# MariusFurter/WeightedSampling.jl

Hardware: NVIDIA B200
Metric: particle_updates_per_sec (higher is better)
Workload: dtype f64

## Files before the change

### weightedsampling.jl_b200/csrc/ws_internal.h

```cpp
#pragma once
#include <cuda_runtime.h>
#include <stdint.h>
#include "ws_vm.cuh"
#include "ws_mailbox.cuh"

#ifndef WS_VM_BLOCK
#define WS_VM_BLOCK 128
#endif
#ifndef WS_VM_P
#define WS_VM_P 3
#endif
#ifndef WS_VM_MINB
#define WS_VM_MINB 5
#endif
#define WS_VM_MAX_IO 24
#define WS_VM_MAX_CKPT 16
#define WS_VM_MAX_OPS 96
#define WS_VM_MAX_REGS ((192 * 1024) / (WS_VM_BLOCK * WS_VM_P * 8))
#define WS_SCAN_BLOCK 256
#define WS_SCAN_ITEMS 8
#define WS_SCAN_TILE (32 * WS_SCAN_ITEMS)
#define WS_CDF_TILE (WS_SCAN_BLOCK * WS_SCAN_ITEMS)
#define WS_GATHER_MAX_PLANES 32
#define WS_HEAVY_TILE_SLOTS 32768
// ... 75 lines not shown

struct WsGatherParams {
    int64_t n;
    const int32_t* ancestors;
    int32_t n_planes;
    int32_t pad;
    const double* src[WS_GATHER_MAX_PLANES];
    double* dst[WS_GATHER_MAX_PLANES];
};

#define WS_COMPOSE_MAX_CHAIN 24
struct WsComposeParams {
    int64_t n;
    int64_t n_rows;
    int32_t n_chain;
    int32_t pad;
    const int32_t* chain[WS_COMPOSE_MAX_CHAIN];
};

cudaError_t ws_launch_vm(const WsVmProgram& P, int grid, cudaStream_t s);
cudaError_t ws_launch_reduce_logw(const double* logw, int64_t n, WsLse* partials, int grid, cudaStream_t s);
cudaError_t ws_launch_finalize(const WsLse* partials, int n_partials, int k, int64_t n_global, double ess_perc_min,
                               WsReduceOut* out, unsigned long long* ties, cudaStream_t s);
#define WS_SMALL_N 4096
cudaError_t ws_launch_resample_small(const WsScanParams& P, const WsLse* partials, int n_partials, double ess_perc_min, WsReduceOut* out,
                                     unsigned long long* ties, int do_finalize, cudaStream_t s);
void ws_scan_set_scale(WsScanParams& P);
size_t ws_scan_words(int64_t n);
cudaError_t ws_launch_scan_search(const WsScanParams& P, int grid, cudaStream_t s);
cudaError_t ws_launch_spacings(const WsScanParams& P, cudaStream_t s);
cudaError_t ws_launch_cdf(const WsScanParams& P, cudaStream_t s);
cudaError_t ws_launch_bounds(const WsScanParams& P, cudaStream_t s);
cudaError_t ws_launch_search(const WsScanParams& P, cudaStream_t s);
cudaError_t ws_launch_finalize_global(const double* all_msq, int n_ranks, int64_t n_global, double ess_perc_min,
                                      WsReduceOut* out, cudaStream_t s, unsigned long long* ties = nullptr);
cudaError_t ws_launch_finalize_mbox(const WsLse* partials, int n_partials, int64_t n_global, double ess_perc_min, WsReduceOut* out,
                                    double* all_msq, unsigned long long* ties, const WsMailbox& M, cudaStream_t s);
cudaError_t ws_launch_cdf_tiles(const WsScanParams& P, cudaStream_t s);
cudaError_t ws_launch_offsets_bounds_mbox(const WsScanParams& P, const WsMailbox& M, unsigned long long* all_tot, const unsigned long long* xmine,
                                          int xw, unsigned long long* xall, cudaStream_t s);
cudaError_t ws_launch_barrier_mbox(const WsMailbox& M, cudaStream_t s);
cudaError_t ws_launch_gather(const WsGatherParams& P, int grid, cudaStream_t s);
cudaError_t ws_launch_fill(double* dst, double v, int64_t n, int grid, cudaStream_t s);
cudaError_t ws_launch_exp_norm(const double* logw, const WsReduceOut* red, double* w, int64_t n, int grid,
                               cudaStream_t s);
cudaError_t ws_launch_sumsq(const double* w, int64_t n, double* partials, int grid, cudaStream_t s);
cudaError_t ws_launch_local_ancestors(int32_t* anc, int64_t n, const int32_t* anc_self, int64_t self_lo, int64_t self_hi,
                                      int64_t spare_base, int grid, cudaStream_t s);
cudaError_t ws_launch_patch_ancestors(int32_t* anc, int64_t n, int64_t self_lo, int64_t self_hi, int64_t spare_base, cudaStream_t s);
struct WsTracedPlane {
    const double* src;
    double* dst;
    int64_t level;
};
cudaError_t ws_launch_trace_rows(const int32_t* anc, int64_t m, const int32_t* const* chain, int n_levels, int64_t n_rows, int32_t* rows,
                                 cudaStream_t s);
cudaError_t ws_launch_push_traced(const WsTracedPlane* planes, int n_planes, int64_t m, const int32_t* rows, cudaStream_t s);
cudaError_t ws_launch_gather_rows(const double* src, const int64_t* idx, int64_t n_idx, double* dst, cudaStream_t s);
cudaError_t ws_launch_compose(const WsComposeParams& P, int32_t* out, const int32_t* start, cudaStream_t s);
cudaError_t ws_launch_compose_rows(const WsComposeParams& P, int64_t* out, const int64_t* start, cudaStream_t s);
int ws_vm_sl_grid(const WsVmProgram& P);
int ws_vm_max_grid(int n_regs, int n_loads, int n_ops, int sm_count, int n_ckpt = 0);
int ws_vm_smem_bytes(int n_regs, int n_loads, int n_ops, int n_ckpt = 0);
cudaError_t ws_kernels_init(int device);
```

### weightedsampling.jl_b200/csrc/ws_kernels.cu

```cuda
#include "ws_internal.h"

static int g_sm_count = 148;

__device__ __forceinline__ void lse_push(WsLse& a, double l) {
    if (l == -INFINITY) return;
    if (l > a.m) {
        double sc = ws_exp_nonpos(a.m - l);
        a.S = a.S * sc + 1.0;
        a.Q = a.Q * sc * sc + 1.0;
        a.m = l;
    } else {
        double e = ws_exp_nonpos(l - a.m);
        a.S += e;
        a.Q += e * e;
    }
}

template <int K>
__device__ __forceinline__ void lse_push_many(WsLse& a, const double (&l)[K], const bool (&live)[K]) {
    double mx = -INFINITY;
#pragma unroll
    for (int j = 0; j < K; ++j)
        if (live[j]) mx = fmax(mx, l[j]);
    if (mx > a.m) {
        const double sc = ws_exp_nonpos(a.m - mx);
        a.S *= sc;
        a.Q *= sc * sc;
        a.m = mx;
    }
#pragma unroll
    for (int j = 0; j < K; ++j) {
        if (live[j] && l[j] != -INFINITY) {
            const double e = ws_exp_nonpos(l[j] - a.m);
// ... 294 lines not shown

    if (P.logw_mode != 0 && P.partials != nullptr) {
        WsLse tot = lse_block_reduce<WS_VM_BLOCK>(part, warp_scratch);
        if (threadIdx.x == 0) P.partials[blockIdx.x] = tot;
    }
    for (int c = 0; CKPT && c < P.n_ckpt; ++c) {
        WsLse st;
        st.m = ck[(c * 3 + 0) * WS_VM_BLOCK];
        st.S = ck[(c * 3 + 1) * WS_VM_BLOCK];
        st.Q = ck[(c * 3 + 2) * WS_VM_BLOCK];
        __syncthreads();
        WsLse tot = lse_block_reduce<WS_VM_BLOCK>(st, warp_scratch);
        if (threadIdx.x == 0) P.ckpt_partials[(size_t)c * gridDim.x + blockIdx.x] = tot;
    }
    if (P.n_expect > 0) {
        __shared__ double esc[WS_VM_BLOCK / 32][8];
        const int lane = threadIdx.x & 31, warp = threadIdx.x >> 5;
#pragma unroll
        for (int k = 0; k < 8; ++k) {
            double v = esum[k];
#pragma unroll
            for (int d = 16; d > 0; d >>= 1) v += __shfl_down_sync(0xffffffffu, v, d);
            if (lane == 0) esc[warp][k] = v;
        }
        __syncthreads();
        if (threadIdx.x < 8 && threadIdx.x < P.n_expect) {
            double v = 0.0;
            for (int w = 0; w < WS_VM_BLOCK / 32; ++w) v += esc[w][threadIdx.x];
            P.expect_partials[(size_t)blockIdx.x * P.n_expect + threadIdx.x] = v;
        }
    }
}

#include "ws_vm_sl.cuh"
#ifndef WS_SL_P
#define WS_SL_P 4
#endif
#ifndef WS_SL_MINB
#define WS_SL_MINB 3
#endif
template <class Sig, int PP>
__global__ void __launch_bounds__(WS_VM_BLOCK, WS_SL_MINB) ws_vm_sl_kernel(const __grid_constant__ WsVmProgram P) {
    extern __shared__ __align__(16) double ws_vm_smem[];
    __shared__ WsLse warp_scratch[WS_VM_BLOCK / 32];
    constexpr int RS = PP * WS_VM_BLOCK;
    constexpr int TILE = WS_VM_BLOCK * PP;
    constexpr int NL = Sig::n_loads, NS = Sig::n_stores;
    double* const stage = ws_vm_smem + threadIdx.x;

    WsLse part;
    part.m = -INFINITY;
    part.S = 0.0;
    part.Q = 0.0;
    const int n = (int)P.n;
    const int n_tiles = (n + TILE - 1) / TILE;
    const bool fired = (P.logw_mode != 3) || P.red->do_resample != 0;
    const int lmode = (P.logw_mode == 3) ? (fired ? 2 : 1) : P.logw_mode;
    const double lbase = (P.logw_mode == 3) ? P.red->log_mean_w : P.logw_base;
    const bool any_gather = P.load_gather != 0u && fired;

    auto tile_index = [&](int tile, int j) -> int {
        const int i = tile * TILE + (int)threadIdx.x + j * WS_VM_BLOCK;
        return i < n ? i : n - 1;
    };
    auto issue_stage = [&](int tile, const int (&anc)[PP]) {
#pragma unroll
        for (int k = 0; k < NL; ++k) {
            const bool g = any_gather && ((P.load_gather >> k) & 1u);
            const double* __restrict__ ptr = P.load_ptr[k];
#pragma unroll
            for (int j = 0; j < PP; ++j)
                ws_cp_async8(stage + k * RS + j * WS_VM_BLOCK, ptr + (unsigned)(g ? anc[j] : tile_index(tile, j)));
        }
        ws_cp_async_commit();
    };
// ... 164 lines not shown
        for (int j = 0; j < PP; ++j)
            if (live[j]) lout[(unsigned)first + j * WS_VM_BLOCK] = lw[j];
    }
#pragma unroll
    for (int c = 0; c < NCK; ++c) {
        if (c < reps) {
            __syncthreads();
            WsLse tot = lse_block_reduce<WS_VM_BLOCK>(st[c], warp_scratch);
            if (threadIdx.x == 0) {
                P.ckpt_partials[(size_t)c * gridDim.x + blockIdx.x] = tot;
                if (c == reps - 1 && P.partials != nullptr) P.partials[blockIdx.x] = tot;
            }
        }
    }
}
static bool ws_slck_ok(const WsVmProgram& P) {
    return P.n_ckpt > 0 && P.n_expect == 0 && (P.logw_mode == 1 || P.logw_mode == 2) && ws_sl_matches_repeated<WsSigLinregObs>(P, WS_SLCK_N);
}
static int ws_slck_grid(const WsVmProgram& P) {
    constexpr int TILE = WS_VM_BLOCK * WS_SLCK_P;
    const int64_t tiles = (P.n + TILE - 1) / TILE;
    const int grid = (int)(tiles < (int64_t)g_sm_count * WS_SLCK_MINB ? tiles : (int64_t)g_sm_count * WS_SLCK_MINB);
    return grid < 1 ? 1 : grid;
}

static bool g_vm_interp_only = false;
template <class Sig>
static cudaError_t ws_launch_vm_sl(const WsVmProgram& P, cudaStream_t s) {
    constexpr int TILE = WS_VM_BLOCK * WS_SL_P;
    const int64_t tiles = (P.n + TILE - 1) / TILE;
    int grid = (int)(tiles < (int64_t)g_sm_count * WS_SL_MINB ? tiles : (int64_t)g_sm_count * WS_SL_MINB);
    if (grid < 1) grid = 1;
    const int smem = (Sig::n_loads > 0 ? Sig::n_loads : 1) * TILE * (int)sizeof(double);
    ws_vm_sl_kernel<Sig, WS_SL_P><<<grid, WS_VM_BLOCK, smem, s>>>(P);
    return cudaGetLastError();
}
int ws_vm_sl_grid(const WsVmProgram& P) {
    if (!g_vm_interp_only && P.n_ckpt != 0 && ws_slck_ok(P)) return ws_slck_grid(P);
    if (g_vm_interp_only || P.n_ckpt != 0 || ws_sl_find(P) < 0) return 0;
    constexpr int TILE = WS_VM_BLOCK * WS_SL_P;
    const int64_t tiles = (P.n + TILE - 1) / TILE;
    int grid = (int)(tiles < (int64_t)g_sm_count * WS_SL_MINB ? tiles : (int64_t)g_sm_count * WS_SL_MINB);
    return grid < 1 ? 1 : grid;
}

static bool ws_vm_staged(int n_regs, int n_loads) {
    return n_loads > 0 && (size_t)(n_regs + n_loads) * WS_VM_BLOCK * WS_VM_P * sizeof(double) <= (size_t)200 * 1024;
}
int ws_vm_smem_bytes(int n_regs, int n_loads, int n_ops, int n_ckpt) {
    const int rows = (n_regs < 1 ? 1 : n_regs) + (ws_vm_staged(n_regs < 1 ? 1 : n_regs, n_loads) ? n_loads : 0);
    return rows * WS_VM_BLOCK * WS_VM_P * (int)sizeof(double) + n_ops * (int)sizeof(WsDop) + n_ckpt * 3 * WS_VM_BLOCK * (int)sizeof(double);
}

int ws_vm_max_grid(int n_regs, int n_loads, int n_ops, int sm_count, int n_ckpt) {
    const int smem = ws_vm_smem_bytes(n_regs, n_loads, n_ops, n_ckpt) + 1024;
    int per_sm = (227 * 1024) / smem;
    if (per_sm > WS_VM_MINB) per_sm = WS_VM_MINB;
    if (per_sm < 1) per_sm = 1;
    return per_sm * sm_count;
}

cudaError_t ws_launch_vm(const WsVmProgram& P, int grid, cudaStream_t s) {
    if (!g_vm_interp_only && P.n_ckpt == 0) {
        switch (ws_sl_find(P)) {
#define WS_SL_CASE(idx, Sig) \
    case idx: return ws_launch_vm_sl<Sig>(P, s);
            WS_SL_SIGS(WS_SL_CASE)
#undef WS_SL_CASE
// ... 5 lines not shown
        ws_vm_sl_ckpt_kernel<WsSigLinregObs, WS_SLCK_P, WS_SLCK_N><<<ws_slck_grid(P), WS_VM_BLOCK, smem_ck, s>>>(P);
        return cudaGetLastError();
    }
    const int smem = ws_vm_smem_bytes(P.n_regs, P.n_loads, P.n_ops, P.n_ckpt);
    if (P.n_ckpt > 0) {
        if (ws_vm_staged(P.n_regs, P.n_loads)) ws_vm_kernel<true, true><<<grid, WS_VM_BLOCK, smem, s>>>(P);
        else ws_vm_kernel<false, true><<<grid, WS_VM_BLOCK, smem, s>>>(P);
    } else if (ws_vm_staged(P.n_regs, P.n_loads)) ws_vm_kernel<true><<<grid, WS_VM_BLOCK, smem, s>>>(P);
    else ws_vm_kernel<false><<<grid, WS_VM_BLOCK, smem, s>>>(P);
    return cudaGetLastError();
}

__global__ void __launch_bounds__(256) ws_reduce_logw_kernel(const double* __restrict__ logw, int64_t n,
                                                             WsLse* __restrict__ partials) {
    __shared__ WsLse warp_scratch[8];
    WsLse part;
    part.m = -INFINITY;
    part.S = 0.0;
    part.Q = 0.0;
    const int64_t stride = (int64_t)gridDim.x * 256;
    for (int64_t i = (int64_t)blockIdx.x * 256 + threadIdx.x; i < n; i += stride) lse_push(part, __ldg(logw + i));
    WsLse tot = lse_block_reduce<256>(part, warp_scratch);
    if (threadIdx.x == 0) partials[blockIdx.x] = tot;
}

cudaError_t ws_launch_reduce_logw(const double* logw, int64_t n, WsLse* partials, int grid, cudaStream_t s) {
    ws_reduce_logw_kernel<<<grid, 256, 0, s>>>(logw, n, partials);
    return cudaGetLastError();
}

__global__ void __launch_bounds__(256) ws_finalize_kernel(const WsLse* __restrict__ partials, int n_partials,
                                                          int64_t n_global, double ess_perc_min,
                                                          WsReduceOut* __restrict__ out, unsigned long long* ties) {
    __shared__ WsLse warp_scratch[8];
    const WsLse tot = lse_block_combine<256>(partials + (size_t)blockIdx.x * n_partials, n_partials, warp_scratch);
    if (threadIdx.x == 0) ws_decide(tot, n_global, ess_perc_min, out + blockIdx.x, ties);
}

cudaError_t ws_launch_finalize(const WsLse* partials, int n_partials, int k, int64_t n_global, double ess_perc_min,
                               WsReduceOut* out, unsigned long long* ties, cudaStream_t s) {
    ws_finalize_kernel<<<k, 256, 0, s>>>(partials, n_partials, n_global, ess_perc_min, out, ties);
    return cudaGetLastError();
}

__global__ void ws_finalize_global_kernel(const double* __restrict__ all_msq, int n_ranks, int64_t n_global,
                                          double ess_perc_min, WsReduceOut* __restrict__ out, unsigned long long* ties) {
    if (threadIdx.x != 0 || blockIdx.x != 0) return;
    ws_decide(lse_combine_ranks(all_msq, n_ranks), n_global, ess_perc_min, out, ties);
}

cudaError_t ws_launch_finalize_global(const double* all_msq, int n_ranks, int64_t n_global, double ess_perc_min,
                                      WsReduceOut* out, cudaStream_t s, unsigned long long* ties) {
    ws_finalize_global_kernel<<<1, 32, 0, s>>>(all_msq, n_ranks, n_global, ess_perc_min, out, ties);
    return cudaGetLastError();
}

__global__ void __launch_bounds__(WS_MBOX_THREADS) ws_finalize_mbox_kernel(const WsLse* __restrict__ partials, int n_partials, int64_t n_global,
                                                                           double ess_perc_min, WsReduceOut* __restrict__ out,
                                                                           double* __restrict__ all_msq, unsigned long long* ties,
                                                                           const __grid_constant__ WsMailbox M) {
    __shared__ WsLse warp_scratch[WS_MBOX_THREADS / 32];
    __shared__ unsigned long long mine[3];
    __shared__ unsigned long long all[3 * WS_MBOX_MAX_RANKS];
    const WsLse loc = lse_block_combine<WS_MBOX_THREADS>(partials, n_partials, warp_scratch);
    if (threadIdx.x == 0) {
        mine[0] = (unsigned long long)__double_as_longlong(loc.m);
        mine[1] = (unsigned long long)__double_as_longlong(loc.S);
        mine[2] = (unsigned long long)__double_as_longlong(loc.Q);
    }
    __syncthreads();
    ws_mbox_allgather(M, M.seq, mine, 3, all);
    if (threadIdx.x != 0) return;
    const double* msq = reinterpret_cast<const double*>(all);
    for (int k = 0; k < 3 * M.nranks; ++k) all_msq[k] = msq[k];
    ws_decide(lse_combine_ranks(msq, M.nranks), n_global, ess_perc_min, out, ties);
// ... 274 lines not shown
        unsigned long long run = carry + warp_excl + (incl - thread_total);
#pragma unroll
        for (int k = 0; k < WS_OFF_ITEMS; ++k) {
            if (i0 + k < n_tiles) words[i0 + k] = run;
            run += v[k];
        }
        __syncthreads();
        if (threadIdx.x == 0) s_carry = carry + total;
        __syncthreads();
    }
    if (threadIdx.x == 0 && total_out != nullptr) *total_out = s_carry;
}
__global__ void __launch_bounds__(1024) ws_cdf_offsets_kernel(const __grid_constant__ WsScanParams P) {
    if (P.gate != 0 && P.red->do_resample == 0) return;
    ws_scan_words_cta(P.tile_words, (int)((P.n + WS_CDF_TILE - 1) / WS_CDF_TILE), P.total);
}
__device__ __forceinline__ void ws_cdf_group_offsets_body(const WsScanParams& P) {
    if (threadIdx.x == 0 && P.heavy_count != nullptr) *P.heavy_count = 0u;
    if (P.gate != 0 && P.red->do_resample == 0) return;
    const int n_tiles = (int)((P.n + WS_CDF_TILE - 1) / WS_CDF_TILE);
    const int n_groups = (n_tiles + WS_TILE_GROUP - 1) / WS_TILE_GROUP;
    unsigned long long* const grp = P.tile_words + n_tiles;
    const int lane = threadIdx.x & 31, warp = threadIdx.x >> 5;
    for (int g = warp; g < n_groups; g += 32) {
        const int idx = g * WS_TILE_GROUP + lane;
        unsigned long long v = idx < n_tiles ? P.tile_words[idx] : 0ull;
#pragma unroll
        for (int d = 16; d > 0; d >>= 1) v += __shfl_xor_sync(0xffffffffu, v, d);
        if (lane == 0) grp[g] = v;
    }
    __syncthreads();
    ws_scan_words_cta(grp, n_groups, P.total);
}
__global__ void __launch_bounds__(1024) ws_cdf_group_offsets_kernel(const __grid_constant__ WsScanParams P) { ws_cdf_group_offsets_body(P); }
__device__ __forceinline__ unsigned long long ws_tile_offset(const WsScanParams& P, const int n_tiles, const int ct, const int lane) {
    const int g = ct / WS_TILE_GROUP, idx = g * WS_TILE_GROUP + lane;
    unsigned long long v = idx < ct ? __ldg(P.tile_words + idx) : 0ull;
    if (lane == 31) v = __ldg(P.tile_words + n_tiles + g);
#pragma unroll
    for (int d = 16; d > 0; d >>= 1) v += __shfl_xor_sync(0xffffffffu, v, d);
    return v;
}

__device__ __forceinline__ unsigned long long ws_mn_threshold(unsigned long long C, unsigned long long S_total) {
    const unsigned long long lo = C * S_total, hi = __umul64hi(C, S_total);
    return (hi << 3) | (lo >> 61);
}
__device__ __forceinline__ unsigned long long ws_mn_block_prefix(const WsScanParams& P, int b) {
    return __ldg(P.mn_tile_off + b / (WS_CDF_TILE / WS_SCAN_TILE)) + __ldg(P.mn_block_local + b);
}
__device__ __forceinline__ int ws_mn_find_block(const WsScanParams& P, unsigned long long T) {
    constexpr int BPT = WS_CDF_TILE / WS_SCAN_TILE;
    const int n_all = (int)P.n_slots + 1;
    const int n_tiles = (n_all + WS_CDF_TILE - 1) / WS_CDF_TILE, n_blocks = (n_all + WS_SCAN_TILE - 1) / WS_SCAN_TILE;
    int lo = 0, hi = n_tiles - 1;
    while (lo < hi) {
        const int mid = (lo + hi + 1) >> 1;
        if (__ldg(P.mn_tile_off + mid) <= T) lo = mid; else hi = mid - 1;
    }
    const unsigned long long base = __ldg(P.mn_tile_off + lo);
    int b = lo * BPT;
    const int b_end = min(b + BPT, n_blocks);
    for (int j = b + 1; j < b_end; ++j)
        if (base + __ldg(P.mn_block_local + j) <= T) b = j;
    return b;
}
__device__ __forceinline__ int ws_F_mn(const WsScanParams& P, unsigned long long C) {
// ... 508 lines not shown
                const int hi = __shfl_sync(0xffffffffu, f[k], src);
                if (hi - lo > WS_DIRECT_MAX) {
                    const int a = max(lo, chunk), e = min(hi, chunk_end);
                    const int anc = tile_base + src * WS_SCAN_ITEMS + k;
                    for (int pos = a + lane; pos < e; pos += 32) out_s[pos - chunk] = anc;
                }
                lo = hi;
            }
        }
        __syncwarp();
        for (int pos = chunk + lane; pos < chunk_end; pos += 32) P.ancestors[pos - slot_base] = out_s[pos - chunk];
        __syncwarp();
    }
}

#ifndef WS_SEARCH_ASYNC
#define WS_SEARCH_ASYNC 1
#endif
#ifndef WS_SEARCH_MINB
#define WS_SEARCH_MINB 3
#endif
#ifndef WS_SEARCH_GRID
#define WS_SEARCH_GRID 3
#endif
__device__ __forceinline__ bool ws_gate_closed_identity(const WsScanParams& P) {
    if (P.gate == 0 || P.red->do_resample != 0) return false;
    const int64_t stride = (int64_t)gridDim.x * blockDim.x;
    for (int64_t i = (int64_t)blockIdx.x * blockDim.x + threadIdx.x; i < P.n; i += stride) P.ancestors[i] = (int32_t)i;
    return true;
}
#define WS_SEARCH_SMEM_BYTES ((WS_WARPS_PER_CTA * WS_RBUF_SLOTS + WS_CDF_TILE) * 8)
template <bool EXACT_FP, bool MN, bool SHR>
__global__ void __launch_bounds__(WS_SCAN_BLOCK, WS_SEARCH_MINB) ws_search_kernel(const __grid_constant__ WsScanParams P) {
    if (ws_gate_closed_identity(P)) return;

    extern __shared__ __align__(16) unsigned long long search_smem[];
    static_assert(WS_RBUF_SLOTS * 8 >= (WS_EXPAND_CHUNK + 128) * 4 && (WS_RBUF_SLOTS * 8) % 16 == 0, "window too small for the offspring staging");
    const int lane = threadIdx.x & 31, warp = threadIdx.x >> 5;
    unsigned long long* const rbuf = search_smem + warp * WS_RBUF_SLOTS;
    ulonglong2* const cbuf = reinterpret_cast<ulonglong2*>(search_smem + WS_WARPS_PER_CTA * WS_RBUF_SLOTS + warp * WS_SCAN_TILE) + lane;

    const unsigned long long cdf_offset = ws_cdf_offset(P);
    WsSearchCtx X;
    ws_search_setup(P, X);
    const int n = X.n;
    const int n_tiles = (n + WS_SCAN_TILE - 1) / WS_SCAN_TILE;
    const int n_ctiles = (n + WS_CDF_TILE - 1) / WS_CDF_TILE;
    const int warps_total = gridDim.x * WS_WARPS_PER_CTA;

#if WS_SEARCH_ASYNC
    unsigned long long ow = 0ull, pw = 0ull;
    auto request = [&](int tile) {
        const int tile_base = tile * WS_SCAN_TILE;
        const int ct = tile_base / WS_CDF_TILE;
        if (tile_base + WS_SCAN_TILE <= n) {
            const ulonglong2* p2 = reinterpret_cast<const ulonglong2*>(P.cdf_local + tile_base + lane * WS_SCAN_ITEMS);
#pragma unroll
            for (int k = 0; k < WS_SCAN_ITEMS / 2; ++k) ws_cp_async16(cbuf + k * 32, p2 + k);
        }
        ws_cp_async_commit();
        const int idx = (ct / WS_TILE_GROUP) * WS_TILE_GROUP + lane;
        ow = idx < ct ? __ldg(P.tile_words + idx) : 0ull;
        if (lane == 31) ow = __ldg(P.tile_words + n_ctiles + ct / WS_TILE_GROUP);
        pw = (lane == 0 && tile_base % WS_CDF_TILE != 0) ? __ldg(P.cdf_local + tile_base - 1) : 0ull;
    };
    static_assert(WS_EXPAND_CHUNK * 4 + WS_RING_BLOCKS * 16 <= WS_RBUF_SLOTS * 8 && 32 * WS_EXPAND_LANE <= WS_EXPAND_CHUNK,
// ... 496 lines not shown
        for (int k = 0; k < WS_SCAN_ITEMS; ++k) {
            const int i = item0 + k;
            if (i < n) {
                int fk = ws_F_int(excl + q[k], (unsigned int)ns, sh, rmask, P.scheme == 1 ? 1 : 0, r0, P.seed, P.stream);
                if (i == n - 1) {
                    if (fk < ns) atomicAdd(P.n_clamped, (unsigned long long)(ns - fk));
                    fk = ns;
                }
                Fs[i] = fk;
            }
        }
        __syncthreads();
        if (threadIdx.x == 0) s_carry += chunk_tot;
    }
    __syncthreads();
    for (int j = threadIdx.x; j < ns; j += 256) {
        int lo = 0, hi = n - 1;
        while (lo < hi) {
            const int mid = (lo + hi) >> 1;
            if (Fs[mid] > j) hi = mid; else lo = mid + 1;
        }
        P.ancestors[j] = lo;
    }
}

cudaError_t ws_launch_resample_small(const WsScanParams& P, const WsLse* partials, int n_partials, double ess_perc_min, WsReduceOut* out,
                                     unsigned long long* ties, int do_finalize, cudaStream_t s) {
    ws_resample_small_kernel<<<1, 256, 0, s>>>(P, partials, n_partials, ess_perc_min, out, ties, do_finalize,
                                               reinterpret_cast<int32_t*>(P.cdf_local));
    return cudaGetLastError();
}

__global__ void __launch_bounds__(256) ws_expand_heavy_kernel(const __grid_constant__ WsScanParams P) {
    if (P.gate != 0 && P.red->do_resample == 0) return;
    __shared__ int32_t Fs[WS_SCAN_TILE];
    const unsigned int n_heavy = *P.heavy_count;
    for (unsigned int h = 0; h < n_heavy; ++h) {
        const int32_t* src = P.heavy_F + (size_t)h * (WS_SCAN_TILE + 2);
        __syncthreads();
        for (int k = threadIdx.x; k < WS_SCAN_TILE; k += 256) Fs[k] = src[k];
        __syncthreads();
        const int64_t fstart = (int64_t)src[WS_SCAN_TILE];
        const int64_t tile_base = (int64_t)src[WS_SCAN_TILE + 1] * WS_SCAN_TILE;
        const int64_t fend = (int64_t)Fs[WS_SCAN_TILE - 1];
        const int64_t len = fend - fstart;
        const int64_t per = (len + gridDim.x - 1) / gridDim.x;
        const int64_t a = fstart + (int64_t)blockIdx.x * per;
        const int64_t e = (a + per < fend) ? a + per : fend;
        for (int64_t j = a + threadIdx.x; j < e; j += 256) {
            int lo = 0, hi = WS_SCAN_TILE - 1;
            while (lo < hi) {
                const int mid = (lo + hi) >> 1;
                if ((int64_t)Fs[mid] > j) hi = mid; else lo = mid + 1;
            }
            P.ancestors[j - P.slot_base] = (int32_t)(tile_base + lo);
        }
    }
}

static int g_fx_extra_bits = 0;
void ws_scan_set_scale(WsScanParams& P) {
    const bool exact_fp = P.replay_u != nullptr || P.sorted_u != nullptr;
    int shift = 61;
    {
        int bits = 0;
        while (((int64_t)1 << bits) < P.n_slots + 1) ++bits;
// ... 1 lines not shown
    }
    if (!exact_fp && P.scheme != 2) {
        int bits = 0;
        while (((int64_t)1 << bits) < P.n_slots) ++bits;
        shift = 61 - bits - g_fx_extra_bits;
        if (shift < 24) shift = 24;
    }
    P.fx_shift = shift;
    P.fx_scale = (exact_fp || P.scheme == 2) ? 2305843009213693952.0 : ldexp((double)P.n_slots, shift);
}

cudaError_t ws_launch_spacings(const WsScanParams& P, cudaStream_t s) {
    const int64_t n_all = P.n_slots + 1;
    const int64_t tiles = (n_all + WS_CDF_TILE - 1) / WS_CDF_TILE;
    int g = (int)(tiles < (int64_t)g_sm_count * 8 ? tiles : (int64_t)g_sm_count * 8);
    ws_spacing_tiles_kernel<<<g < 1 ? 1 : g, WS_SCAN_BLOCK, 0, s>>>(P);
    cudaError_t e = cudaGetLastError();
    if (e != cudaSuccess) return e;
    WsScanParams Q = P;
    Q.n = n_all;
    Q.tile_words = P.mn_tile_off;
    Q.total = P.mn_total;
    ws_cdf_offsets_kernel<<<1, 1024, 0, s>>>(Q);
    return cudaGetLastError();
}

cudaError_t ws_launch_cdf(const WsScanParams& P, cudaStream_t s) {
    const int64_t cdf_tiles = (P.n + WS_CDF_TILE - 1) / WS_CDF_TILE;
    int g1 = (int)(cdf_tiles < (int64_t)g_sm_count * WS_CDF_GRID ? cdf_tiles : (int64_t)g_sm_count * WS_CDF_GRID);
    if (g1 < 1) g1 = 1;
    ws_cdf_tiles_kernel<<<g1, WS_SCAN_BLOCK, 0, s>>>(P);
    cudaError_t e = cudaGetLastError();
    if (e != cudaSuccess) return e;
    ws_cdf_group_offsets_kernel<<<1, 1024, 0, s>>>(P);
    return cudaGetLastError();
}

cudaError_t ws_launch_bounds(const WsScanParams& P, cudaStream_t s) {
    const bool exact_fp = P.replay_u != nullptr || P.sorted_u != nullptr;
    if (exact_fp) ws_bounds_kernel<true><<<1, 32, 0, s>>>(P);
    else ws_bounds_kernel<false><<<1, 32, 0, s>>>(P);
    return cudaGetLastError();
}

cudaError_t ws_launch_cdf_tiles(const WsScanParams& P, cudaStream_t s) {
    const int64_t cdf_tiles = (P.n + WS_CDF_TILE - 1) / WS_CDF_TILE;
    int g1 = (int)(cdf_tiles < (int64_t)g_sm_count * WS_CDF_GRID ? cdf_tiles : (int64_t)g_sm_count * WS_CDF_GRID);
    if (g1 < 1) g1 = 1;
    ws_cdf_tiles_kernel<<<g1, WS_SCAN_BLOCK, 0, s>>>(P);
    return cudaGetLastError();
}
cudaError_t ws_launch_offsets_bounds_mbox(const WsScanParams& P, const WsMailbox& M, unsigned long long* all_tot, const unsigned long long* xmine,
                                          int xw, unsigned long long* xall, cudaStream_t s) {
    const bool exact_fp = P.replay_u != nullptr || P.sorted_u != nullptr;
    if (exact_fp) ws_offsets_bounds_mbox_kernel<true><<<1, 1024, 0, s>>>(P, M, all_tot, xmine, xw, xall);
    else ws_offsets_bounds_mbox_kernel<false><<<1, 1024, 0, s>>>(P, M, all_tot, xmine, xw, xall);
    return cudaGetLastError();
}

cudaError_t ws_launch_search(const WsScanParams& P, cudaStream_t s) {
    const int64_t warp_tiles = (P.n + WS_SCAN_TILE - 1) / WS_SCAN_TILE;
    const int64_t ctas = (warp_tiles + WS_WARPS_PER_CTA - 1) / WS_WARPS_PER_CTA;
    int g3 = (int)(ctas < (int64_t)g_sm_count * WS_SEARCH_GRID ? ctas : (int64_t)g_sm_count * WS_SEARCH_GRID);
    if (g3 < 1) g3 = 1;
    const bool exact_fp = P.replay_u != nullptr || P.sorted_u != nullptr;
    if (exact_fp) ws_search_kernel<true, false, false><<<g3, WS_SCAN_BLOCK, WS_SEARCH_SMEM_BYTES, s>>>(P);
    else if (P.scheme == 2) ws_search_kernel<false, true, false><<<g3, WS_SCAN_BLOCK, WS_SEARCH_SMEM_BYTES, s>>>(P);
    else if (P.fx_shift >= 32) ws_search_kernel<false, false, true><<<g3, WS_SCAN_BLOCK, WS_SEARCH_SMEM_BYTES, s>>>(P);
    else ws_search_kernel<false, false, false><<<g3, WS_SCAN_BLOCK, WS_SEARCH_SMEM_BYTES, s>>>(P);
    cudaError_t e = cudaGetLastError();
    if (e != cudaSuccess) return e;
    ws_expand_heavy_kernel<<<g_sm_count * 4, 256, 0, s>>>(P);
    return cudaGetLastError();
}

#ifndef WS_SCAN_DEFAULT_FORM
#define WS_SCAN_DEFAULT_FORM 0
#endif
static int g_scan_form = WS_SCAN_DEFAULT_FORM;
#ifndef WS_CHAIN_DEFAULT_BLOCK
#define WS_CHAIN_DEFAULT_BLOCK WS_SCAN_BLOCK
#endif
static int g_chain_block = WS_CHAIN_DEFAULT_BLOCK;
template <int BLOCK>
static cudaError_t ws_launch_chain(const WsScanParams& P, bool exact_fp, cudaStream_t s) {
    const int64_t tiles = (P.n + BLOCK * WS_SCAN_ITEMS - 1) / (BLOCK * WS_SCAN_ITEMS);
    const int64_t resident = (int64_t)g_sm_count * WS_CHAIN_MINB * (WS_SCAN_BLOCK / BLOCK);
    int g = (int)(tiles < resident ? tiles : resident);
    if (g < 1) g = 1;
    if (exact_fp) ws_chain_kernel<true, BLOCK><<<g, BLOCK, WS_CHAIN_SMEM_BYTES(BLOCK), s>>>(P);
    else ws_chain_kernel<false, BLOCK><<<g, BLOCK, WS_CHAIN_SMEM_BYTES(BLOCK), s>>>(P);
    return cudaGetLastError();
}
cudaError_t ws_launch_scan_search(const WsScanParams& P, int grid, cudaStream_t s) {
    (void)grid;
    if (g_scan_form != 0 && P.all_tot == nullptr && P.total == nullptr && P.bounds == nullptr && P.scheme != 2) {
        const int64_t cdf_tiles = (P.n + WS_CDF_TILE - 1) / WS_CDF_TILE;
        const bool exact_fp = P.replay_u != nullptr || P.sorted_u != nullptr;
        cudaError_t e = cudaMemsetAsync(P.tile_counter, 0, sizeof(unsigned int) * 2, s);
        if (e != cudaSuccess) return e;
        if (g_scan_form == 2) {
            const int64_t ch_tiles = (P.n + g_chain_block * WS_SCAN_ITEMS - 1) / (g_chain_block * WS_SCAN_ITEMS);
            e = cudaMemsetAsync(P.tile_words, 0, sizeof(unsigned long long) * (size_t)(ch_tiles + 3 * ((ch_tiles + WS_CHAIN_GROUP - 1) / WS_CHAIN_GROUP)), s);
            if (e != cudaSuccess) return e;
            e = g_chain_block == 32 ? ws_launch_chain<32>(P, exact_fp, s) : (g_chain_block == 64 ? ws_launch_chain<64>(P, exact_fp, s) : ws_launch_chain<WS_SCAN_BLOCK>(P, exact_fp, s));
            if (e != cudaSuccess) return e;
        } else {
// ... 231 lines not shown
```

### weightedsampling.jl_b200/csrc/ws_runtime.cu

```cuda
#include <math.h>
#include <stdarg.h>
#include <stdio.h>
#include <string.h>
#include <algorithm>
#include <functional>
#include <memory>
#include <deque>
#include <map>
#include <string>
#include <vector>

#include <dlfcn.h>
#include <unistd.h>
#include <chrono>

#include "../../include/wsb200.h"
#include "ws_internal.h"
#include "ws_lowering.h"
#include "ws_move.h"
#include "ws_stats.h"
#include "ws_exchange.h"

using wsl::Plane;
using wsl::Program;
// ... 250 lines not shown
};

static int materialize_planes(ws_ctx* c, const std::vector<Plane>* only = nullptr);
static int materialize_deep(ws_ctx* c, const std::vector<Plane>& planes);
static int map_for_epoch(ws_ctx* c, int64_t ep, const int32_t** out);
static const int32_t* anc_of_event(const ws_ctx* c, int64_t event);
static int materialize_tape_planes(ws_ctx* c, int32_t n_extra, const int32_t* col, const int32_t* comp);
static int resolve_spec(ws_ctx* c);
static int mbox_setup(ws_ctx* c);
static WsMailbox mbox_next(ws_ctx* c, int n_exchanges);
static int mbox_check(ws_ctx* c);

static int fail(ws_ctx* c, int code, const char* fmt, ...) {
    char buf[1024];
    va_list ap;
    va_start(ap, fmt);
    vsnprintf(buf, sizeof(buf), fmt, ap);
    va_end(ap);
    if (c != nullptr) c->err = buf; else g_create_error = buf;
    return code;
}
#define CK(c, call)                                                                                     \
    do {                                                                                                \
        cudaError_t e__ = (call);                                                                       \
        if (e__ != cudaSuccess)                                                                         \
            return fail((c), e__ == cudaErrorMemoryAllocation ? WS_ENOMEM : WS_ECUDA, "%s failed: %s (%s:%d)", #call, \
                        cudaGetErrorString(e__), __FILE__, __LINE__);                                   \
    } while (0)
#define TRY(expr)                 \
    do {                          \
        int rc__ = (expr);        \
        if (rc__ != WS_OK) return rc__; \
    } while (0)
#define NCK(c, call)                                                                                       \
    do {                                                                                                   \
        int r__ = (call);                                                                                  \
        if (r__ != 0) return fail((c), WS_ENCCL, "%s failed: %s", #call, g_nccl.GetErrorString(r__));      \
    } while (0)

static void timed_begin(ws_ctx* c, int kclass, TimedEvent& te) {
    te.kclass = kclass;
    te.a = te.b = nullptr;
    c->stats.kernel_launches++;
    c->kc_count[kclass]++;
    if (!c->timing) return;
    if (c->event_pool.empty()) {
        cudaEventCreate(&te.a);
        cudaEventCreate(&te.b);
    } else {
        te.a = c->event_pool.back().first;
        te.b = c->event_pool.back().second;
        c->event_pool.pop_back();
    }
    cudaEventRecord(te.a, c->stream);
}
static void timed_end(ws_ctx* c, TimedEvent& te) {
    if (!c->timing || te.a == nullptr) return;
    cudaEventRecord(te.b, c->stream);
    c->pending_events.push_back(te);
}
static void resolve_events(ws_ctx* c) {
    if (c->pending_events.empty()) return;
    cudaStreamSynchronize(c->stream);
    for (auto& te : c->pending_events) {
        float ms = 0.f;
        if (cudaEventElapsedTime(&ms, te.a, te.b) == cudaSuccess) c->kc_ms[te.kclass] += (double)ms;
// ... 398 lines not shown
    }
    if (w.has_acc) {
        P.logw = c->logw;
        if (c->logw_spec) {
            P.logw_mode = 3;
            P.red = c->d_red;
        } else if (c->logw_uniform) {
            P.logw_mode = 2;
            P.logw_base = c->logw_base;
        } else {
            P.logw_mode = 1;
        }
    } else {
        P.logw_mode = 0;
    }
    if (c->spec_flushing) {
        P.n_ckpt = (int32_t)c->spec_steps.size();
        for (int32_t j = 0; j < P.n_ckpt; ++j) P.ckpt_pc[j] = (uint8_t)c->spec_steps[j].ckpt_pc;
        P.ckpt_partials = c->d_ck_partials;
        P.logw_out = c->d_logw_bak;
    }
    const int64_t vm_tile = (int64_t)WS_VM_BLOCK * WS_VM_P;
    const int grid = (int)std::min<int64_t>(ws_vm_max_grid(P.n_regs, P.n_loads, P.n_ops, c->sm_count, P.n_ckpt), (c->n + vm_tile - 1) / vm_tile);
    P.partials = w.has_acc ? c->d_partials : nullptr;
    P.n_expect = 0;
    P.rng.seed = c->seed;
    P.rng.replay_n = c->d_replay_n;
    P.rng.replay_u = c->d_replay_u;
    P.rng.replay_e = c->d_replay_e;
    P.rng.replay_v = c->d_replay_v;
    memcpy(P.ops, w.ops.data(), sizeof(WsOp) * w.ops.size());

    const int sl_grid = ws_vm_sl_grid(P);
    TimedEvent te;
    timed_begin(c, KC_VM, te);
    CK(c, ws_launch_vm(P, std::max(1, grid), c->stream));
    timed_end(c, te);
    if (sl_grid > 0) c->stats.sl_passes++;
    for (auto& pl : swap_after) std::swap(c->cols[pl.col].front[pl.comp], c->cols[pl.col].back[pl.comp]);
    for (auto& pl : w.dirty) {
        c->cols[pl.col].stale[pl.comp] = 0;
        c->cols[pl.col].ep[pl.comp] = c->epoch;
    }
    c->stats.fused_passes++;
    c->stats.fused_statements += w.n_statements;
    if (w.has_acc) {
        c->logw_uniform = false;
        c->logw_spec = false;
        c->partials_valid = true;
        c->n_partials = sl_grid > 0 ? sl_grid : std::max(1, grid);
        c->red_valid = false;
    }
    reset_window(c);
    return WS_OK;
}

extern "C" int ws_flush(ws_ctx* c) {
    if (!c) return WS_EINVAL;
    return flush_window(c);
}
extern "C" int ws_sync(ws_ctx* c) {
    if (!c) return WS_EINVAL;
    TRY(flush_window(c));
    CK(c, cudaStreamSynchronize(c->stream));
    TRY(resolve_spec(c));
    return WS_OK;
// ... 881 lines not shown
        }
        const size_t slots = (size_t)(n / WS_HEAVY_TILE_SLOTS) + 2;
        CK(c, cudaMalloc(&c->d_heavy_F, sizeof(int32_t) * slots * (WS_SCAN_TILE + 2)));
        c->heavy_cap_n = n;
    }
    (void)n_tiles;
    WsScanParams S;
    memset(&S, 0, sizeof(S));
    S.logw = d_w;
    S.mode = mode;
    S.scheme = scheme;
    S.red = c->d_red;
    S.gate = gate;
    S.n = n;
    S.n_slots = n;
    S.cdf_offset = 0ull;
    S.slot_base = 0;
    S.last_rank = 1;
    S.bounds = nullptr;
    S.total = nullptr;
    S.seed = c->seed;
    S.stream = stream_id;
    S.replay_u = d_replay_u;
    S.sorted_u = d_sorted_u;
    S.ancestors = d_anc;
    S.tile_words = d_words;
    S.cdf_local = d_cdf_local;
    S.tile_counter = c->d_tile_counter;
    S.n_clamped = d_clamped;
    S.heavy_count = c->d_tile_counter + 1;
    S.heavy_F = c->d_heavy_F;
    ws_scan_set_scale(S);
    if (scheme == WS_RESAMPLER_MULTINOMIAL && d_sorted_u == nullptr && d_replay_u == nullptr) TRY(prepare_multinomial(c, S));
    TimedEvent te;
    timed_begin(c, KC_SCAN, te);
    CK(c, ws_launch_scan_search(S, 0, c->stream));
    c->stats.kernel_launches += 3;
    timed_end(c, te);
    return WS_OK;
}

static int allgather_host_bytes(ws_ctx* c, const void* mine, size_t bytes, std::vector<char>& all) {
    const size_t R = (size_t)c->nranks, words = bytes / 8;
    TRY(ensure_scratch2(c, bytes * (R + 1)));
    char* d = (char*)c->d_scratch2;
    CK(c, cudaMemcpyAsync(d + bytes * R, mine, bytes, cudaMemcpyHostToDevice, c->stream));
    NCK(c, g_nccl.AllGather(d + bytes * R, d, words, WS_NCCL_UINT64, c->comm, c->stream));
    all.resize(bytes * R);
    CK(c, cudaMemcpyAsync(all.data(), d, bytes * R, cudaMemcpyDeviceToHost, c->stream));
    CK(c, cudaStreamSynchronize(c->stream));
    return WS_OK;
}

static WsMailbox mbox_next(ws_ctx* c, int n_exchanges) {
    WsMailbox M;
    memset(&M, 0, sizeof(M));
    for (int q = 0; q < c->nranks; ++q) M.box[q] = c->mbox_peer[(size_t)q];
    M.rank = c->rank;
    M.nranks = c->nranks;
    M.seq = c->mbox_seq + 1u;
    M.cap = c->mbox_cap;
    M.err = c->d_mbox_err;
    M.timeout_ns = 60000000000ull;
    if (const char* e = getenv("WSB200_MAILBOX_TIMEOUT_MS")) M.timeout_ns = strtoull(e, nullptr, 10) * 1000000ull;
    c->mbox_seq += (uint32_t)n_exchanges;
    c->mbox_exchanges += n_exchanges;
// ... 1930 lines not shown
    return WS_OK;
}
extern "C" int ws_next_philox_stream(ws_ctx* c, uint64_t* stream_out, uint64_t* seed_out) {
    if (!c) return WS_EINVAL;
    if (stream_out) *stream_out = c->next_stream;
    if (seed_out) *seed_out = c->seed;
    return WS_OK;
}
extern "C" int ws_get_traced_pushes(ws_ctx* c, int64_t* out) {
    if (!c || !out) return WS_EINVAL;
    *out = c->traced_rows;
    return WS_OK;
}
extern "C" int ws_get_mailbox_exchanges(ws_ctx* c, int64_t* out) {
    if (!c || !out) return WS_EINVAL;
    *out = c->mbox_on ? c->mbox_exchanges : 0;
    return WS_OK;
}
extern "C" int ws_get_pushed(ws_ctx* c, int64_t* out) {
    if (!c || !out) return WS_EINVAL;
    *out = c->pushed_total;
    return WS_OK;
}
extern "C" int ws_get_migrated(ws_ctx* c, int64_t* out) {
    if (!c || !out) return WS_EINVAL;
    *out = c->migrated_total;
    return WS_OK;
}
extern "C" int ws_stream(ws_ctx* c, void** stream_out) {
    if (!c || !stream_out) return WS_EINVAL;
    *stream_out = (void*)c->stream;
    return WS_OK;
}
```

Measured before the change: 44.91 billion.

## Launch dependent kernels with programmatic dependent launch and add overlap probe

Launches the single-launch VM, finalize, CDF group-offsets, search and heavy-expand kernels through cudaLaunchKernelEx with programmatic stream serialization. Each of these kernels now begins with griddepcontrol.wait followed by launch_dependents, so the next kernel's launch and prologue can overlap the tail of the previous one. The aim is to hide per-kernel launch latency across the resampling chain. Separately, it adds a compile-time-gated probe that times search and VM kernels concurrently on two streams, which is inactive by default.

New measurement: 44.96 billion, median of 6. About the same (+0.1%).

```diff
diff --git a/weightedsampling.jl_b200/csrc/ws_internal.h b/weightedsampling.jl_b200/csrc/ws_internal.h
--- a/weightedsampling.jl_b200/csrc/ws_internal.h
+++ b/weightedsampling.jl_b200/csrc/ws_internal.h
@@ -131,6 +131,9 @@
 cudaError_t ws_launch_cdf(const WsScanParams& P, cudaStream_t s);
 cudaError_t ws_launch_bounds(const WsScanParams& P, cudaStream_t s);
 cudaError_t ws_launch_search(const WsScanParams& P, cudaStream_t s);
+#ifdef WS_OVERLAP_PROBE
+cudaError_t ws_launch_search_probe(const WsScanParams& P, int ctas_per_sm, cudaStream_t s);
+#endif
 cudaError_t ws_launch_finalize_global(const double* all_msq, int n_ranks, int64_t n_global, double ess_perc_min,
                                       WsReduceOut* out, cudaStream_t s, unsigned long long* ties = nullptr);
 cudaError_t ws_launch_finalize_mbox(const WsLse* partials, int n_partials, int64_t n_global, double ess_perc_min, WsReduceOut* out,
diff --git a/weightedsampling.jl_b200/csrc/ws_kernels.cu b/weightedsampling.jl_b200/csrc/ws_kernels.cu
--- a/weightedsampling.jl_b200/csrc/ws_kernels.cu
+++ b/weightedsampling.jl_b200/csrc/ws_kernels.cu
@@ -1,4 +1,5 @@
 #include "ws_internal.h"
+#include <utility>
 
 static int g_sm_count = 148;
 
@@ -359,6 +360,24 @@
     }
 }
 
+__device__ __forceinline__ void ws_pdl_enter() {
+    asm volatile("griddepcontrol.wait;\n\tgriddepcontrol.launch_dependents;" ::: "memory");
+}
+template <typename... KArgs, typename... Args>
+static cudaError_t ws_launch_pdl(void (*kernel)(KArgs...), dim3 grid, dim3 block, size_t smem, cudaStream_t s, Args&&... args) {
+    cudaLaunchConfig_t cfg = {};
+    cfg.gridDim = grid;
+    cfg.blockDim = block;
+    cfg.dynamicSmemBytes = smem;
+    cfg.stream = s;
+    cudaLaunchAttribute at[1];
+    at[0].id = cudaLaunchAttributeProgrammaticStreamSerialization;
+    at[0].val.programmaticStreamSerializationAllowed = 1;
+    cfg.attrs = at;
+    cfg.numAttrs = 1;
+    return cudaLaunchKernelEx(&cfg, kernel, std::forward<Args>(args)...);
+}
+
 #include "ws_vm_sl.cuh"
 #ifndef WS_SL_P
 #define WS_SL_P 4
@@ -368,6 +387,7 @@
 #endif
 template <class Sig, int PP>
 __global__ void __launch_bounds__(WS_VM_BLOCK, WS_SL_MINB) ws_vm_sl_kernel(const __grid_constant__ WsVmProgram P) {
+    ws_pdl_enter();
     extern __shared__ __align__(16) double ws_vm_smem[];
     __shared__ WsLse warp_scratch[WS_VM_BLOCK / 32];
     constexpr int RS = PP * WS_VM_BLOCK;
@@ -598,8 +618,7 @@
     int grid = (int)(tiles < (int64_t)g_sm_count * WS_SL_MINB ? tiles : (int64_t)g_sm_count * WS_SL_MINB);
     if (grid < 1) grid = 1;
     const int smem = (Sig::n_loads > 0 ? Sig::n_loads : 1) * TILE * (int)sizeof(double);
-    ws_vm_sl_kernel<Sig, WS_SL_P><<<grid, WS_VM_BLOCK, smem, s>>>(P);
-    return cudaGetLastError();
+    return ws_launch_pdl(ws_vm_sl_kernel<Sig, WS_SL_P>, dim3(grid), dim3(WS_VM_BLOCK), smem, s, P);
 }
 int ws_vm_sl_grid(const WsVmProgram& P) {
     if (!g_vm_interp_only && P.n_ckpt != 0 && ws_slck_ok(P)) return ws_slck_grid(P);
@@ -671,6 +690,7 @@
 __global__ void __launch_bounds__(256) ws_finalize_kernel(const WsLse* __restrict__ partials, int n_partials,
                                                           int64_t n_global, double ess_perc_min,
                                                           WsReduceOut* __restrict__ out, unsigned long long* ties) {
+    ws_pdl_enter();
     __shared__ WsLse warp_scratch[8];
     const WsLse tot = lse_block_combine<256>(partials + (size_t)blockIdx.x * n_partials, n_partials, warp_scratch);
     if (threadIdx.x == 0) ws_decide(tot, n_global, ess_perc_min, out + blockIdx.x, ties);
@@ -678,8 +698,7 @@
 
 cudaError_t ws_launch_finalize(const WsLse* partials, int n_partials, int k, int64_t n_global, double ess_perc_min,
                                WsReduceOut* out, unsigned long long* ties, cudaStream_t s) {
-    ws_finalize_kernel<<<k, 256, 0, s>>>(partials, n_partials, n_global, ess_perc_min, out, ties);
-    return cudaGetLastError();
+    return ws_launch_pdl(ws_finalize_kernel, dim3(k), dim3(256), 0, s, partials, n_partials, n_global, ess_perc_min, out, ties);
 }
 
 __global__ void ws_finalize_global_kernel(const double* __restrict__ all_msq, int n_ranks, int64_t n_global,
@@ -1020,7 +1039,10 @@
     __syncthreads();
     ws_scan_words_cta(grp, n_groups, P.total);
 }
-__global__ void __launch_bounds__(1024) ws_cdf_group_offsets_kernel(const __grid_constant__ WsScanParams P) { ws_cdf_group_offsets_body(P); }
+__global__ void __launch_bounds__(1024) ws_cdf_group_offsets_kernel(const __grid_constant__ WsScanParams P) {
+    ws_pdl_enter();
+    ws_cdf_group_offsets_body(P);
+}
 __device__ __forceinline__ unsigned long long ws_tile_offset(const WsScanParams& P, const int n_tiles, const int ct, const int lane) {
     const int g = ct / WS_TILE_GROUP, idx = g * WS_TILE_GROUP + lane;
     unsigned long long v = idx < ct ? __ldg(P.tile_words + idx) : 0ull;
@@ -1595,6 +1617,7 @@
 #define WS_SEARCH_SMEM_BYTES ((WS_WARPS_PER_CTA * WS_RBUF_SLOTS + WS_CDF_TILE) * 8)
 template <bool EXACT_FP, bool MN, bool SHR>
 __global__ void __launch_bounds__(WS_SCAN_BLOCK, WS_SEARCH_MINB) ws_search_kernel(const __grid_constant__ WsScanParams P) {
+    ws_pdl_enter();
     if (ws_gate_closed_identity(P)) return;
 
     extern __shared__ __align__(16) unsigned long long search_smem[];
@@ -2157,6 +2180,7 @@
 }
 
 __global__ void __launch_bounds__(256) ws_expand_heavy_kernel(const __grid_constant__ WsScanParams P) {
+    ws_pdl_enter();
     if (P.gate != 0 && P.red->do_resample == 0) return;
     __shared__ int32_t Fs[WS_SCAN_TILE];
     const unsigned int n_heavy = *P.heavy_count;
@@ -2224,8 +2248,7 @@
     ws_cdf_tiles_kernel<<<g1, WS_SCAN_BLOCK, 0, s>>>(P);
     cudaError_t e = cudaGetLastError();
     if (e != cudaSuccess) return e;
-    ws_cdf_group_offsets_kernel<<<1, 1024, 0, s>>>(P);
-    return cudaGetLastError();
+    return ws_launch_pdl(ws_cdf_group_offsets_kernel, dim3(1), dim3(1024), 0, s, P);
 }
 
 cudaError_t ws_launch_bounds(const WsScanParams& P, cudaStream_t s) {
@@ -2250,21 +2273,24 @@
     return cudaGetLastError();
 }
 
-cudaError_t ws_launch_search(const WsScanParams& P, cudaStream_t s) {
+static cudaError_t ws_launch_search_at(const WsScanParams& P, int ctas_per_sm, bool heavy, cudaStream_t s) {
     const int64_t warp_tiles = (P.n + WS_SCAN_TILE - 1) / WS_SCAN_TILE;
     const int64_t ctas = (warp_tiles + WS_WARPS_PER_CTA - 1) / WS_WARPS_PER_CTA;
-    int g3 = (int)(ctas < (int64_t)g_sm_count * WS_SEARCH_GRID ? ctas : (int64_t)g_sm_count * WS_SEARCH_GRID);
+    int g3 = (int)(ctas < (int64_t)g_sm_count * ctas_per_sm ? ctas : (int64_t)g_sm_count * ctas_per_sm);
     if (g3 < 1) g3 = 1;
     const bool exact_fp = P.replay_u != nullptr || P.sorted_u != nullptr;
-    if (exact_fp) ws_search_kernel<true, false, false><<<g3, WS_SCAN_BLOCK, WS_SEARCH_SMEM_BYTES, s>>>(P);
-    else if (P.scheme == 2) ws_search_kernel<false, true, false><<<g3, WS_SCAN_BLOCK, WS_SEARCH_SMEM_BYTES, s>>>(P);
-    else if (P.fx_shift >= 32) ws_search_kernel<false, false, true><<<g3, WS_SCAN_BLOCK, WS_SEARCH_SMEM_BYTES, s>>>(P);
-    else ws_search_kernel<false, false, false><<<g3, WS_SCAN_BLOCK, WS_SEARCH_SMEM_BYTES, s>>>(P);
-    cudaError_t e = cudaGetLastError();
-    if (e != cudaSuccess) return e;
-    ws_expand_heavy_kernel<<<g_sm_count * 4, 256, 0, s>>>(P);
-    return cudaGetLastError();
-}
+    void (*kernel)(WsScanParams) = exact_fp ? ws_search_kernel<true, false, false>
+                                   : P.scheme == 2 ? ws_search_kernel<false, true, false>
+                                   : P.fx_shift >= 32 ? ws_search_kernel<false, false, true>
+                                   : ws_search_kernel<false, false, false>;
+    cudaError_t e = ws_launch_pdl(kernel, dim3(g3), dim3(WS_SCAN_BLOCK), WS_SEARCH_SMEM_BYTES, s, P);
+    if (e != cudaSuccess || !heavy) return e;
+    return ws_launch_pdl(ws_expand_heavy_kernel, dim3(g_sm_count * 4), dim3(256), 0, s, P);
+}
+cudaError_t ws_launch_search(const WsScanParams& P, cudaStream_t s) { return ws_launch_search_at(P, WS_SEARCH_GRID, true, s); }
+#ifdef WS_OVERLAP_PROBE
+cudaError_t ws_launch_search_probe(const WsScanParams& P, int ctas_per_sm, cudaStream_t s) { return ws_launch_search_at(P, ctas_per_sm, false, s); }
+#endif
 
 #ifndef WS_SCAN_DEFAULT_FORM
 #define WS_SCAN_DEFAULT_FORM 0
diff --git a/weightedsampling.jl_b200/csrc/ws_runtime.cu b/weightedsampling.jl_b200/csrc/ws_runtime.cu
--- a/weightedsampling.jl_b200/csrc/ws_runtime.cu
+++ b/weightedsampling.jl_b200/csrc/ws_runtime.cu
@@ -306,6 +306,11 @@
         int rc__ = (expr);        \
         if (rc__ != WS_OK) return rc__; \
     } while (0)
+#ifdef WS_OVERLAP_PROBE
+static WsScanParams g_probe_scan;
+static WsVmProgram g_probe_vm;
+static bool g_probe_have_scan = false, g_probe_have_vm = false;
+#endif
 #define NCK(c, call)                                                                                       \
     do {                                                                                                   \
         int r__ = (call);                                                                                  \
@@ -770,6 +775,12 @@
     memcpy(P.ops, w.ops.data(), sizeof(WsOp) * w.ops.size());
 
     const int sl_grid = ws_vm_sl_grid(P);
+#ifdef WS_OVERLAP_PROBE
+    if (sl_grid > 0 && P.load_gather != 0u) {
+        g_probe_vm = P;
+        g_probe_have_vm = true;
+    }
+#endif
     TimedEvent te;
     timed_begin(c, KC_VM, te);
     CK(c, ws_launch_vm(P, std::max(1, grid), c->stream));
@@ -1717,6 +1728,10 @@
     S.heavy_F = c->d_heavy_F;
     ws_scan_set_scale(S);
     if (scheme == WS_RESAMPLER_MULTINOMIAL && d_sorted_u == nullptr && d_replay_u == nullptr) TRY(prepare_multinomial(c, S));
+#ifdef WS_OVERLAP_PROBE
+    g_probe_scan = S;
+    g_probe_have_scan = true;
+#endif
     TimedEvent te;
     timed_begin(c, KC_SCAN, te);
     CK(c, ws_launch_scan_search(S, 0, c->stream));
@@ -3713,3 +3728,45 @@
     *stream_out = (void*)c->stream;
     return WS_OK;
 }
+
+#ifdef WS_OVERLAP_PROBE
+extern "C" int ws_overlap_probe(ws_ctx* c, int mode, int search_ctas_per_sm, int reps, float* ms_out) {
+    if (!c || !g_probe_have_scan || !g_probe_have_vm || reps < 1 || mode < 0 || mode > 3 || search_ctas_per_sm < 1) return WS_EINVAL;
+    static int32_t* anc = nullptr;
+    static int64_t anc_n = 0;
+    static cudaStream_t s2 = nullptr;
+    static cudaEvent_t e0, e1, es;
+    if (s2 == nullptr) {
+        CK(c, cudaStreamCreateWithFlags(&s2, cudaStreamNonBlocking));
+        CK(c, cudaEventCreate(&e0));
+        CK(c, cudaEventCreate(&e1));
+        CK(c, cudaEventCreateWithFlags(&es, cudaEventDisableTiming));
+    }
+    if (anc_n < g_probe_scan.n) {
+        CK(c, cudaStreamSynchronize(c->stream));
+        if (anc) CK(c, cudaFree(anc));
+        CK(c, cudaMalloc(&anc, sizeof(int32_t) * (size_t)g_probe_scan.n));
+        anc_n = g_probe_scan.n;
+    }
+    WsScanParams S = g_probe_scan;
+    S.ancestors = anc;
+    for (int r = 0; r < reps; ++r) {
+        CK(c, cudaMemsetAsync(S.tile_counter, 0, sizeof(unsigned int) * 2, c->stream));
+        CK(c, cudaEventRecord(e0, c->stream));
+        if (mode == 1) {
+            CK(c, cudaStreamWaitEvent(s2, e0, 0));
+            CK(c, ws_launch_search_probe(S, search_ctas_per_sm, s2));
+            CK(c, cudaEventRecord(es, s2));
+            CK(c, ws_launch_vm(g_probe_vm, 1, c->stream));
+            CK(c, cudaStreamWaitEvent(c->stream, es, 0));
+        } else {
+            if (mode != 3) CK(c, ws_launch_search_probe(S, search_ctas_per_sm, c->stream));
+            if (mode != 2) CK(c, ws_launch_vm(g_probe_vm, 1, c->stream));
+        }
+        CK(c, cudaEventRecord(e1, c->stream));
+        CK(c, cudaEventSynchronize(e1));
+        CK(c, cudaEventElapsedTime(ms_out + r, e0, e1));
+    }
+    return WS_OK;
+}
+#endif
```
